# martinhoT/Footsies-Gym

Hardware: NVIDIA B200
Metric: env_frames_per_sec (higher is better)
Workload: dtype int32+fp32

## Files before the change

footsies_gym_b200/_capi.py:

```python
import ctypes as C
import os

from . import build as _build

FG_STATE_PLANES = 4
FG_STAT_COUNT = 16
STAT_NAMES = ["episodes", "p1_wins", "p2_wins", "double_ko", "episode_frames", "p1_specials",
              "p1_specials_neutral", "guard_breaks", "hits", "blocks", "env_frames", "resets"]


class FgConfig(C.Structure):
    _fields_ = [("struct_size", C.c_int32), ("num_envs", C.c_int32), ("device", C.c_int32),
                ("p1_bot", C.c_int32), ("p2_bot", C.c_int32), ("dense_reward", C.c_int32),
                ("frame_skip", C.c_int32), ("autoreset", C.c_int32), ("stale_intro_input", C.c_int32),
                ("skip_unactionable", C.c_int32), ("first_env_index", C.c_int64)]


class FgBuffers(C.Structure):
    _fields_ = [("struct_size", C.c_int32), ("reserved0", C.c_int32),
                ("state", C.c_void_p * FG_STATE_PLANES), ("stats", C.c_void_p),
                ("actions_p1", C.c_void_p), ("actions_p2", C.c_void_p), ("obs", C.c_void_p),
                ("reward", C.c_void_p), ("terminated", C.c_void_p), ("info_frame", C.c_void_p),
                ("info_misc", C.c_void_p), ("step_mask", C.c_void_p)]

# ... 70 lines not shown
        lib = load()
        self.nbytes = int(nbytes)
        ptr = lib.fg_host_alloc(int(device_index), self.nbytes)
        if not ptr:
            raise FootsiesLibraryError("fg_host_alloc failed: " + lib.fg_last_error().decode("utf-8", "replace"))
        self.ptr = ptr
        raw = (C.c_uint8 * max(self.nbytes, 1)).from_address(ptr)
        weakref.finalize(raw, lib.fg_host_free, ptr).atexit = False
        self.bytes = torch.frombuffer(raw, dtype=torch.uint8, count=self.nbytes)
        self._offset = 0

    def take(self, shape, dtype):
        import torch
        n = int(torch.Size(shape).numel()) * torch.empty((), dtype=dtype).element_size()
        off = (self._offset + 63) // 64 * 64
        if off + n > self.nbytes:
            raise ValueError("host block exhausted")
        self._offset = off + n
        return self.bytes[off:off + n].view(dtype).reshape(shape)


_lib = None

EXPORTS = ["fg_abi_version", "fg_last_error", "fg_algorithmic_bytes_per_env_step", "fg_create", "fg_destroy",
           "fg_bind", "fg_seed", "fg_reset", "fg_step", "fg_step_host", "fg_reset_host", "fg_step_host_compact",
           "fg_reset_host_compact", "fg_packed_reward_table", "fg_step_host_packed", "fg_reset_host_packed", "fg_host_alloc",
           "fg_host_free", "fg_delay_ring_step", "fg_get_state",
           "fg_set_state", "fg_read_stats", "fg_launch_count", "fg_policy_mlp_sample", "fg_policy_mlp_sample_p2", "fg_policy_last_error",
           "fg_rollout_mlp", "fg_rollout_mlp_pool", "fg_value_mlp", "fg_gae"]


def load(build_if_missing=True):
    global _lib
    if _lib is not None:
        return _lib
    path = _build.LIB_PATH
    if os.environ.get("FOOTSIES_B200_LIB"):
        pass
    elif _build.is_stale(path):
        if not build_if_missing:
            raise FootsiesLibraryError(f"{path} is missing or stale: run `python -m footsies_gym_b200.build`")
        _build.build()
    L = C.CDLL(path)
    vp, i32, i64 = C.c_void_p, C.c_int32, C.c_int64
    L.fg_abi_version.restype = i32
    L.fg_last_error.restype = C.c_char_p
    L.fg_algorithmic_bytes_per_env_step.restype = i32
    L.fg_algorithmic_bytes_per_env_step.argtypes = [C.POINTER(FgConfig)]
    L.fg_create.restype = i32
    L.fg_create.argtypes = [C.POINTER(FgConfig), C.POINTER(vp)]
    L.fg_destroy.restype = None
    L.fg_destroy.argtypes = [vp]
    L.fg_bind.restype = i32
    L.fg_bind.argtypes = [vp, C.POINTER(FgBuffers)]
    L.fg_seed.restype = i32
    L.fg_seed.argtypes = [vp, i64, vp, vp]
    L.fg_reset.restype = i32
    L.fg_reset.argtypes = [vp, vp, vp]
    L.fg_step.restype = i32
    L.fg_step.argtypes = [vp, vp]
    L.fg_step_host.restype = i32
    L.fg_step_host.argtypes = [vp, vp, vp, vp, vp, vp, vp, vp, vp]
    L.fg_reset_host.restype = i32
    L.fg_reset_host.argtypes = [vp, vp, vp, vp, vp, vp]
    L.fg_step_host_compact.restype = i32
    L.fg_step_host_compact.argtypes = [vp, vp, vp, C.POINTER(FgHostOutputs), vp]
    L.fg_reset_host_compact.restype = i32
    L.fg_reset_host_compact.argtypes = [vp, vp, C.POINTER(FgHostOutputs), vp]
    L.fg_packed_reward_table.restype = i32
    L.fg_packed_reward_table.argtypes = [vp, vp, vp]
    L.fg_step_host_packed.restype = i32
# ... 41 lines not shown
```

footsies_gym_b200/csrc/footsies_kernels.cu:

```cuda
#include <sched.h>
#include <stdlib.h>
#include <algorithm>

#include "rollout_kernel.h"
#include "step_kernel.cuh"

using namespace fg;
using namespace fgk;

namespace {

thread_local char g_err[512] = "";
int fail(int code, const char *fmt, const char *detail = "") {
    snprintf(g_err, sizeof g_err, fmt, detail);
    return code;
}
#define CUDA_TRY(expr) do { cudaError_t _e = (expr); if (_e != cudaSuccess) \
    return fail(FG_ERR_CUDA, #expr ": %s", cudaGetErrorString(_e)); } while (0)

}

struct fg_handle {
    fg_config cfg;
    fg_buffers buf;
// ... 11 lines not shown
    float *d_reward_table;
    uint32_t *d_pack_error;
    float h_reward_table[FG_PACKED_REWARD_TABLE_SIZE];
    int reward_table_count;
    float2 *d_position;
    uint8_t *d_obs_u8;
    cudaStream_t s_compute, s_copy;
    cudaEvent_t ev_fork, ev_join;
    std::vector<cudaEvent_t> ev_slice;
};

namespace {

int grid_for(const fg_handle *h, int blocks_per_sm) {
    int want = (h->cfg.num_envs + kThreads - 1) / kThreads;
    int cap = h->sm_count * blocks_per_sm;
    return want < cap ? (want > 0 ? want : 1) : cap;
}

Params make_params(const fg_handle *h, int first = 0, int count = -1) {
    Params p;
    memset(&p, 0, sizeof p);
    const size_t o = (size_t)first;
    p.pl_f1 = (uint4 *)h->buf.state[FG_PLANE_F1] + o; p.pl_f2 = (uint4 *)h->buf.state[FG_PLANE_F2] + o;
    p.pl_env = (uint4 *)h->buf.state[FG_PLANE_ENV] + o; p.pl_rng = (uint4 *)h->buf.state[FG_PLANE_RNG] + o;
    p.stats = (unsigned long long *)h->buf.stats;
    p.act1 = h->buf.actions_p1 ? h->buf.actions_p1 + o : nullptr;
    p.act2 = h->buf.actions_p2 ? h->buf.actions_p2 + o : nullptr;
    p.obs = (float4 *)h->buf.obs + 2 * o; p.reward = h->buf.reward + o; p.terminated = h->buf.terminated + o;
    p.info_frame = h->buf.info_frame + o; p.info_misc = (uint32_t *)h->buf.info_misc + o;
    p.step_mask = h->buf.step_mask ? h->buf.step_mask + o : nullptr;
    p.tables = h->d_tables;
    p.first_env_index = h->cfg.first_env_index + first;
    p.reverse = (int)(h->step_calls & 1);
    p.pdl = (count < 0 ? h->cfg.num_envs - first : count) >= h->pdl_min_envs;
    p.n = count < 0 ? h->cfg.num_envs - first : count; p.frame_skip = h->cfg.frame_skip; p.autoreset = h->cfg.autoreset;
    p.stale_intro = h->cfg.stale_intro_input;
    p.skip_unactionable = h->cfg.skip_unactionable;
    p.large_shape_min_envs = h->large_shape_min_envs;
    return p;
}

template <bool KF>
cudaError_t launch_step_k(const fg_config &c, int sm_count, cudaStream_t s, const Params &p) {
    const bool d = c.dense_reward != 0, m = p.step_mask != nullptr;
    if (c.p1_bot && c.p2_bot) return launch_step_d<KF, true, true>(d, m, sm_count, s, p);
    if (c.p1_bot) return launch_step_d<KF, true, false>(d, m, sm_count, s, p);
    if (c.p2_bot) return launch_step_d<KF, false, true>(d, m, sm_count, s, p);
// ... 407 lines not shown
    if (int rc = packed_init(h)) return rc;
    memcpy(table, h->h_reward_table, sizeof h->h_reward_table);
    *count = h->reward_table_count;
    return FG_OK;
}
int32_t fg_step_host_packed(fg_handle *h, const uint8_t *a1, const uint8_t *a2, fg_packed_result *out, void *stream) {
    return host_step_packed(h, a1, a2, out, (cudaStream_t)stream);
}
int32_t fg_reset_host_packed(fg_handle *h, const uint8_t *mask, fg_packed_result *out, void *stream) {
    return host_reset_packed(h, mask, out, (cudaStream_t)stream);
}

int32_t fg_abi_version(void) { return FG_ABI_VERSION; }
const char *fg_last_error(void) { return g_err; }

int32_t fg_algorithmic_bytes_per_env_step(const fg_config *cfg) {
    if (!cfg) return 0;
    const bool rng = cfg->p1_bot || cfg->p2_bot;
    int state = 2 * 16 * (rng ? 4 : 3);
    int actions = (cfg->p1_bot ? 0 : 1) + (cfg->p2_bot ? 0 : 1);
    return state + actions + 32  + 4  + 1  + 4  + 4 ;
}

int32_t fg_create(const fg_config *cfg, fg_handle **out) {
    if (!cfg || !out) return fail(FG_ERR_INVALID_ARGUMENT, "null argument%s");
    if (cfg->struct_size != (int32_t)sizeof(fg_config)) return fail(FG_ERR_INVALID_ARGUMENT, "fg_config.struct_size mismatch%s");
    if (cfg->num_envs <= 0) return fail(FG_ERR_INVALID_ARGUMENT, "num_envs must be positive%s");
    if (cfg->frame_skip < 1 || cfg->frame_skip > 64) return fail(FG_ERR_INVALID_ARGUMENT, "frame_skip must be in [1, 64]%s");
    if (cfg->skip_unactionable && cfg->p1_bot) return fail(FG_ERR_INVALID_ARGUMENT, "skip_unactionable needs an agent-controlled P1%s");
    int ndev = 0;
    if (cudaGetDeviceCount(&ndev) != cudaSuccess || ndev == 0) {
        cudaGetLastError();
        return fail(FG_ERR_NO_DEVICE, "no CUDA device: this library has no CPU fallback%s");
    }
    if (cfg->device < 0 || cfg->device >= ndev) return fail(FG_ERR_INVALID_ARGUMENT, "device ordinal out of range%s");
    CUDA_TRY(cudaSetDevice(cfg->device));
    fg_handle *h = new (std::nothrow) fg_handle();
    if (!h) return fail(FG_ERR_INVALID_STATE, "out of host memory%s");
    h->cfg = *cfg;
    h->bound = false;
    h->launches = 0;
    h->step_calls = 0;
    h->d_mask = nullptr;
    h->d_position = nullptr; h->d_obs_u8 = nullptr;
    h->d_packed = nullptr; h->d_reward_table = nullptr; h->d_pack_error = nullptr; h->reward_table_count = 0;
    h->s_compute = h->s_copy = nullptr;
// ... 91 lines not shown
int32_t fg_reset_host(fg_handle *h, const uint8_t *mask, float *obs, int32_t *info_frame, uint8_t *info_misc, void *stream) {
    HostOut o = { obs, nullptr, nullptr, nullptr, nullptr, info_frame, info_misc };
    return host_reset(h, mask, o, (cudaStream_t)stream);
}

int32_t fg_reset_host_compact(fg_handle *h, const uint8_t *mask, const fg_host_outputs *out, void *stream) {
    if (!out || out->struct_size != (int32_t)sizeof(fg_host_outputs))
        return fail(FG_ERR_INVALID_ARGUMENT, "fg_host_outputs is null or its struct_size does not match%s");
    HostOut o = { nullptr, out->position, out->obs_u8, nullptr, nullptr, out->info_frame, out->info_misc };
    return host_reset(h, mask, o, (cudaStream_t)stream);
}

int32_t fg_get_state(fg_handle *h, int32_t first, int32_t count, fg_env_state *out) {
    if (int rc = check_bound(h)) return rc;
    if (!out || first < 0 || count < 0 || (int64_t)first + count > h->cfg.num_envs)
        return fail(FG_ERR_INVALID_ARGUMENT, "env range out of bounds%s");
    CUDA_TRY(cudaSetDevice(h->cfg.device));
    CUDA_TRY(cudaDeviceSynchronize());
    std::vector<FgVec4> pl[FG_STATE_PLANES];
    for (int k = 0; k < FG_STATE_PLANES; k++) {
        pl[k].resize((size_t)count);
        CUDA_TRY(cudaMemcpy(pl[k].data(), (const FgVec4 *)h->buf.state[k] + first, sizeof(FgVec4) * (size_t)count, cudaMemcpyDeviceToHost));
    }
    for (int i = 0; i < count; i++)
        fg_decode_env(pl[FG_PLANE_F1][i], pl[FG_PLANE_F2][i], pl[FG_PLANE_ENV][i], pl[FG_PLANE_RNG][i], &out[i]);
    return FG_OK;
}

int32_t fg_set_state(fg_handle *h, int32_t first, int32_t count, const fg_env_state *in) {
    if (int rc = check_bound(h)) return rc;
    if (!in || first < 0 || count < 0 || (int64_t)first + count > h->cfg.num_envs)
        return fail(FG_ERR_INVALID_ARGUMENT, "env range out of bounds%s");
    std::vector<FgVec4> pl[FG_STATE_PLANES];
    for (int k = 0; k < FG_STATE_PLANES; k++) pl[k].resize((size_t)count);
    for (int i = 0; i < count; i++)
        if (fg_encode_env(&in[i], &pl[FG_PLANE_F1][i], &pl[FG_PLANE_F2][i], &pl[FG_PLANE_ENV][i], &pl[FG_PLANE_RNG][i]))
            return fail(FG_ERR_INVALID_STATE, "state not representable (unknown action id, WIN/has_won, or field out of range)%s");
    CUDA_TRY(cudaSetDevice(h->cfg.device));
    CUDA_TRY(cudaDeviceSynchronize());
    for (int k = 0; k < FG_STATE_PLANES; k++)
        CUDA_TRY(cudaMemcpy((FgVec4 *)h->buf.state[k] + first, pl[k].data(), sizeof(FgVec4) * (size_t)count, cudaMemcpyHostToDevice));
    return FG_OK;
}

int32_t fg_read_stats(fg_handle *h, uint64_t *out, void *stream) {
    if (int rc = check_bound(h)) return rc;
    if (!out) return fail(FG_ERR_INVALID_ARGUMENT, "null output%s");
    CUDA_TRY(cudaSetDevice(h->cfg.device));
    CUDA_TRY(cudaMemcpyAsync(out, h->buf.stats, sizeof(uint64_t) * FG_STAT_COUNT, cudaMemcpyDeviceToHost, (cudaStream_t)stream));
    CUDA_TRY(cudaStreamSynchronize((cudaStream_t)stream));
    return FG_OK;
}

int32_t fg_delay_ring_step(fg_handle *h, int32_t depth, int32_t pos, float *ring_obs, int32_t *ring_frame, uint8_t *ring_misc,
                           float *out_obs, int32_t *out_frame, uint8_t *out_misc, void *stream) {
    if (int rc = check_bound(h)) return rc;
    if (depth < 2 || pos < 0 || pos >= depth) return fail(FG_ERR_INVALID_ARGUMENT, "depth must be frame_delay + 1 >= 2 and 0 <= pos < depth%s");
    if (!ring_obs || !ring_frame || !ring_misc || !out_obs || !out_frame || !out_misc) return fail(FG_ERR_INVALID_ARGUMENT, "null buffer%s");
    if (((uintptr_t)ring_obs & 15u) || ((uintptr_t)out_obs & 15u) || ((uintptr_t)ring_misc & 3u) || ((uintptr_t)out_misc & 3u))
        return fail(FG_ERR_INVALID_ARGUMENT, "obs buffers must be 16-byte, misc buffers 4-byte aligned%s");
// ... 101 lines not shown
```

footsies_gym_b200/csrc/state_codec.h:

```cpp
#ifndef FOOTSIES_B200_STATE_CODEC_H
#define FOOTSIES_B200_STATE_CODEC_H

#include <stdint.h>
#include "../../include/footsies_b200.h"
#include "frame_tables.h"

#if defined(__CUDACC__)
#define FG_HD __host__ __device__ __forceinline__
#else
#define FG_HD static inline
#endif

#define FG_PLANE_F1 0
#define FG_PLANE_F2 1
#define FG_PLANE_ENV 2
#define FG_PLANE_RNG 3

#define FGP_FRAME_SHIFT 0
#define FGP_ACT_SHIFT 6
#define FGP_STUN_SHIFT 11
#define FGP_GUARD_SHIFT 16
#define FGP_VITAL_SHIFT 18
#define FGP_HITCNT_SHIFT 19
#define FGP_BUF_SHIFT 20
#define FGP_RSV_SHIFT 21
#define FGP_INBACK_SHIFT 22
#define FGP_RPROX_SHIFT 23
#define FGP_SHAKE_SHIFT 24
#define FGP_SHAKE_SIGN_SHIFT 27
#define FGP_CARRY_END (1u << 28)
#define FGP_CARRY_ALWAYS (1u << 29)
#define FGP_CARRY_NORMAL (1u << 30)
#define FGP_CARRY_MASK (7u << 28)
#define FGP_ROW_MASK 0x7ffu
#define FGP_MAX_FRAME 63

#define FGH_DASH_SHIFT 0
#define FGH_ARUN_SHIFT 8
// ... 106 lines not shown
    o->frame = (int32_t)e.x;
    o->recorded_input[0] = (int)fg_bits(m, FGM_REC1_SHIFT, 3);
    o->recorded_input[1] = (int)fg_bits(m, FGM_REC2_SHIFT, 3);
    o->done = (int)fg_bits(m, FGM_DONE_SHIFT, 1);
    o->cum_reward_index = (int)fg_bits(m, FGM_CUM_SHIFT, 4);
    o->actor_input[0] = (int)fg_bits(m, FGM_ACTOR1_SHIFT, 3);
    o->actor_input[1] = (int)fg_bits(m, FGM_ACTOR2_SHIFT, 3);
    o->rng_state[0] = r.x; o->rng_state[1] = r.y; o->rng_state[2] = r.z; o->rng_state[3] = r.w;
    o->bot_queue[0] = e.w; o->bot_queue[1] = e.z;
    o->p1_bot_memory = (int)fg_bits(m, FGM_P1MEM_SHIFT, 9);
}

static inline int fg_encode_env(const fg_env_state *s, FgVec4 *f1, FgVec4 *f2, FgVec4 *e, FgVec4 *r) {
    if (fg_encode_fighter(&s->f[0], f1) || fg_encode_fighter(&s->f[1], f2)) return -1;
    if (s->cum_reward_index < 0 || s->cum_reward_index >= FT_NUM_CUM) return -1;
    uint32_t m = ((uint32_t)s->recorded_input[0] & 7u) << FGM_REC1_SHIFT | ((uint32_t)s->recorded_input[1] & 7u) << FGM_REC2_SHIFT
               | (uint32_t)(s->done != 0) << FGM_DONE_SHIFT | (uint32_t)s->cum_reward_index << FGM_CUM_SHIFT
               | ((uint32_t)s->actor_input[0] & 7u) << FGM_ACTOR1_SHIFT | ((uint32_t)s->actor_input[1] & 7u) << FGM_ACTOR2_SHIFT
               | ((uint32_t)s->p1_bot_memory & 0x1ffu) << FGM_P1MEM_SHIFT;
    e->x = (uint32_t)s->frame; e->y = m; e->z = s->bot_queue[1]; e->w = s->bot_queue[0];
    r->x = s->rng_state[0]; r->y = s->rng_state[1]; r->z = s->rng_state[2]; r->w = s->rng_state[3];
    return 0;
}
#endif
```

footsies_gym_b200/csrc/step_kernel.cuh:

```cuda
#ifndef FOOTSIES_B200_STEP_KERNEL_CUH
#define FOOTSIES_B200_STEP_KERNEL_CUH
#include "device_once.h"
#include <cuda_runtime.h>
#include <stdint.h>
#include <stdio.h>
#include <string.h>
#include <new>
#include <vector>

#include "tables_host.h"

namespace fgk {

using namespace fg;

template <int THREADS_, int GROUP_, int STAGES_, int MIN_BLOCKS_>
struct StepShape {
    static constexpr int kThreads = THREADS_, kGroupThreads = GROUP_, kGroups = THREADS_ / GROUP_, kStages = STAGES_,
                         kMinBlocks = MIN_BLOCKS_;
    static_assert(THREADS_ % GROUP_ == 0 && GROUP_ % 32 == 0, "groups are whole warps");
};
#if defined(FG_THREADS)
#ifndef FG_GROUP
#define FG_GROUP FG_THREADS
// ... 2 lines not shown
#define FG_STAGES 2
#endif
#ifndef FG_BLOCKS_PER_SM
#define FG_BLOCKS_PER_SM 4
#endif
using ShapeSmall = StepShape<FG_THREADS, FG_GROUP, FG_STAGES, FG_BLOCKS_PER_SM>;
using ShapeLargeSingle = ShapeSmall;
using ShapeLargeFused = ShapeSmall;
#else
using ShapeSmall = StepShape<256, 256, 2, 3>;
using ShapeLargeSingle = StepShape<768, 256, 3, 1>;
using ShapeLargeFused = StepShape<1024, 256, 3, 1>;
#endif
constexpr int kLargeShapeMinEnvs = 768 * 1024;
#ifndef FG_SKIP_RNG_STORE
#define FG_SKIP_RNG_STORE 1
#endif
#ifndef FG_PDL
#define FG_PDL 1
#endif
#ifndef FG_REVERSE
#define FG_REVERSE 1
#endif
constexpr int kThreads = 256;
constexpr uint32_t kFull = 0xffffffffu;

struct Params {
    uint4 *pl_f1, *pl_f2, *pl_env, *pl_rng;
    unsigned long long *stats;
    const uint8_t *act1, *act2;
    float4 *obs;
    float *reward;
    uint8_t *terminated;
    int32_t *info_frame;
    uint32_t *info_misc;
    const Tables *tables;
    const uint8_t *mask;
    const uint8_t *step_mask;
    long long seed_base, first_env_index;
    int n, frame_skip, autoreset, stale_intro;
    int skip_unactionable;
    int large_shape_min_envs;
    int reverse;
    int pdl;
    int pdl_min_envs;
};

__device__ __forceinline__ void write_outputs(const Params &p, int i, const Env &e, float reward, bool terminated) {
    StepOutputs o;
    make_outputs(e, o);
    p.obs[2 * (size_t)i] = make_float4(o.obs[0], o.obs[1], o.obs[2], o.obs[3]);
    p.obs[2 * (size_t)i + 1] = make_float4(o.obs[4], o.obs[5], o.obs[6], o.obs[7]);
    p.reward[i] = reward;
    p.terminated[i] = terminated ? 1 : 0;
    p.info_frame[i] = e.frame;
    p.info_misc[i] = o.info_misc;
}

__device__ __forceinline__ void load_tables(Tables *dst, const Tables *src) {
    const uint4 *s = reinterpret_cast<const uint4 *>(src);
    uint4 *d = reinterpret_cast<uint4 *>(dst);
    for (int k = threadIdx.x; k < (int)(sizeof(Tables) / 16); k += blockDim.x) d[k] = s[k];
}

template <bool WITH_RNG>
__device__ __forceinline__ void load_env(const Params &p, int i, Env &e) {
    const uint4 a = p.pl_f1[i], b = p.pl_f2[i], c = p.pl_env[i];
    e.pos1 = u2f(a.x); e.vel1 = u2f(a.y); e.pk1 = a.z; e.hist1 = a.w;
    e.pos2 = u2f(b.x); e.vel2 = u2f(b.y); e.pk2 = b.z; e.hist2 = b.w;
    e.frame = (int32_t)c.x; e.misc = c.y; e.bq2 = c.z; e.bq1 = c.w;
    if (WITH_RNG) { const uint4 r = p.pl_rng[i]; e.r0 = r.x; e.r1 = r.y; e.r2 = r.z; e.r3 = r.w; }
    e.drew = false;
}
template <bool WITH_RNG>
__device__ __forceinline__ void store_env(const Params &p, int i, const Env &e) {
    p.pl_f1[i] = make_uint4(f2u(e.pos1), f2u(e.vel1), e.pk1, e.hist1);
    p.pl_f2[i] = make_uint4(f2u(e.pos2), f2u(e.vel2), e.pk2, e.hist2);
    p.pl_env[i] = make_uint4((uint32_t)e.frame, e.misc, e.bq2, e.bq1);
    if (WITH_RNG && (!FG_SKIP_RNG_STORE || e.drew)) p.pl_rng[i] = make_uint4(e.r0, e.r1, e.r2, e.r3);
}

__device__ __forceinline__ void flush_stats(StatAcc &acc, unsigned long long *s_stats, int lane) {
    const uint32_t w[3] = { acc.a, acc.r, acc.s };
    const int map[3][4] = { { FG_STAT_EPISODES, FG_STAT_P1_WINS, FG_STAT_P2_WINS, FG_STAT_DOUBLE_KO },
                            { -1, FG_STAT_HITS, FG_STAT_BLOCKS, FG_STAT_GUARD_BREAKS },
                                            { FG_STAT_P1_SPECIALS, FG_STAT_P1_SPECIALS_NEUTRAL, FG_STAT_RESETS, FG_STAT_ENV_FRAMES } };
#pragma unroll
    for (int k = 0; k < 3; k++)
#pragma unroll
        for (int b = 0; b < 4; b++) {
            if (map[k][b] < 0) continue;
            const uint32_t tot = __reduce_add_sync(kFull, (w[k] >> (8 * b)) & 255u);
            if (lane == 0 && tot) atomicAdd(&s_stats[map[k][b]], (unsigned long long)tot);
        }
    const uint32_t lo = __reduce_add_sync(kFull, acc.ep_frames & 0xffffu), hi = __reduce_add_sync(kFull, acc.ep_frames >> 16);
    if (lane == 0 && (lo | hi)) atomicAdd(&s_stats[FG_STAT_EPISODE_FRAMES], ((unsigned long long)hi << 16) + lo);
    acc.a = 0u; acc.r = 0u; acc.s = 0u; acc.ep_frames = 0u;
}

__device__ __forceinline__ uint32_t smem_u32(const void *p) { return (uint32_t)__cvta_generic_to_shared(p); }
__device__ __forceinline__ void mbar_init(uint64_t *bar, uint32_t count) {
    asm volatile("mbarrier.init.shared::cta.b64 [%0], %1;" ::"r"(smem_u32(bar)), "r"(count));
// ... 3 lines not shown
}
__device__ __forceinline__ void mbar_arrive(uint64_t *bar) {
    asm volatile("mbarrier.arrive.shared::cta.b64 _, [%0];" ::"r"(smem_u32(bar)) : "memory");
}
__device__ __forceinline__ void mbar_wait(uint64_t *bar, uint32_t parity) {
    asm volatile(
        "{\n"
        ".reg .pred P1;\n"
        "LAB_WAIT:\n"
        "mbarrier.try_wait.parity.shared::cta.b64 P1, [%0], %1;\n"
        "@P1 bra DONE;\n"
        "bra LAB_WAIT;\n"
        "DONE:\n"
        "}" ::"r"(smem_u32(bar)), "r"(parity) : "memory");
}
__device__ __forceinline__ void tma_load_1d(void *dst, const void *src, uint32_t bytes, uint64_t *bar) {
    asm volatile("cp.async.bulk.shared::cluster.global.mbarrier::complete_tx::bytes [%0], [%1], %2, [%3];"
                 ::"r"(smem_u32(dst)), "l"(src), "r"(bytes), "r"(smem_u32(bar)) : "memory");
}

template <class SH, int PLANES>
struct __align__(128) StepSmem {
    Tables T;
    uint4 stage[SH::kGroups][SH::kStages][PLANES][SH::kGroupThreads];
    uint64_t full_bar[SH::kGroups][SH::kStages], empty_bar[SH::kGroups][SH::kStages];
    unsigned long long stats[FG_STAT_COUNT];
};

template <class SH, bool KFUSED, bool P1BOT, bool P2BOT, bool DENSE, bool MASKED>
__global__ void __launch_bounds__(SH::kThreads, SH::kMinBlocks) step_kernel(const Params p) {
    constexpr bool kRng = P1BOT || P2BOT;
    constexpr int kPlanes = kRng ? 4 : 3;
    constexpr int kGroupThreads = SH::kGroupThreads, kGroups = SH::kGroups, kStages = SH::kStages;
    extern __shared__ __align__(128) unsigned char smem_raw[];
    StepSmem<SH, kPlanes> &S = *reinterpret_cast<StepSmem<SH, kPlanes> *>(smem_raw);
    const Tables &T = S.T;
    const int lane = threadIdx.x & 31;
    const int g = threadIdx.x / kGroupThreads, lt = threadIdx.x % kGroupThreads;
    const int num_chunks = (p.n + kGroupThreads - 1) / kGroupThreads;
    const int full_chunks = p.n / kGroupThreads;
    const int first = blockIdx.x * kGroups + g, stride = gridDim.x * kGroups;
    const uint4 *const planes[4] = { p.pl_f1, p.pl_f2, p.pl_env, p.pl_rng };
    auto issue = [&](int chunk, int s) {
        mbar_expect_tx(&S.full_bar[g][s], (uint32_t)(kPlanes * kGroupThreads * sizeof(uint4)));
#pragma unroll
        for (int k = 0; k < kPlanes; k++)
            tma_load_1d(S.stage[g][s][k], planes[k] + (size_t)chunk * kGroupThreads, (uint32_t)(kGroupThreads * sizeof(uint4)),
                        &S.full_bar[g][s]);
    };
    auto chunk_of = [&](int c) { return (FG_REVERSE && p.reverse && c < full_chunks) ? full_chunks - 1 - c : c; };
    if (lt == 0) {
        for (int s = 0; s < kStages; s++) { mbar_init(&S.full_bar[g][s], 1u); mbar_init(&S.empty_bar[g][s], kGroupThreads / 32); }
        asm volatile("fence.mbarrier_init.release.cluster;" ::: "memory");
    }
    if (FG_PDL && p.pdl) {
        load_tables(&S.T, p.tables);
        if (threadIdx.x < FG_STAT_COUNT) S.stats[threadIdx.x] = 0ull;
        asm volatile("griddepcontrol.launch_dependents;" ::: "memory");
        asm volatile("griddepcontrol.wait;" ::: "memory");
    }
    if (lt == 0) {
        for (int j = 0; j < kStages - 1; j++) {
            const int cj = first + j * stride;
            if (cj < num_chunks && chunk_of(cj) < full_chunks) issue(chunk_of(cj), j);
        }
    }
    if (!(FG_PDL && p.pdl)) {
        load_tables(&S.T, p.tables);
        if (threadIdx.x < FG_STAT_COUNT) S.stats[threadIdx.x] = 0ull;
    }
    __syncthreads();
    StatAcc acc = { 0u, 0u, 0u, 0u };
    uint32_t frames_since_flush = 0u;
    uint32_t nin1 = 0u, nin2 = 0u;
    {
        const int i0 = (first < num_chunks ? chunk_of(first) : num_chunks) * kGroupThreads + lt;
        if (i0 < p.n) { if (!P1BOT) nin1 = p.act1[i0]; if (!P2BOT) nin2 = p.act2[i0]; }
    }
    int k = 0;
    for (int cl = first; cl < num_chunks; cl += stride, k++) {
        const int s = k % kStages;
        const int c = chunk_of(cl);
        const int i = c * kGroupThreads + lt;
        const bool staged = c < full_chunks;
        bool valid = staged || i < p.n;
        if (MASKED) valid = valid && p.step_mask[valid ? i : 0] != 0;
        if (lt == 0) {
            const int cn = cl + (kStages - 1) * stride;
            if (cn < num_chunks && chunk_of(cn) < full_chunks) {
                const int sn = (k + kStages - 1) % kStages;
                if (k >= 1) mbar_wait(&S.empty_bar[g][sn], ((k - 1) / kStages) & 1);
                issue(chunk_of(cn), sn);
            }
        }
        const uint32_t act1 = nin1, act2 = nin2;
        {
            const int cn1 = cl + stride;
            const int in = (cn1 < num_chunks ? chunk_of(cn1) : num_chunks) * kGroupThreads + lt;
            if (in < p.n) { if (!P1BOT) nin1 = p.act1[in]; if (!P2BOT) nin2 = p.act2[in]; }
        }
        Env e;
        bool run = false;
        uint32_t in1 = 0u, in2 = 0u;
        if (staged) {
            mbar_wait(&S.full_bar[g][s], (k / kStages) & 1);
            const uint4 a = S.stage[g][s][0][lt], b = S.stage[g][s][1][lt], cc = S.stage[g][s][2][lt];
            e.pos1 = u2f(a.x); e.vel1 = u2f(a.y); e.pk1 = a.z; e.hist1 = a.w;
            e.pos2 = u2f(b.x); e.vel2 = u2f(b.y); e.pk2 = b.z; e.hist2 = b.w;
            e.frame = (int32_t)cc.x; e.misc = cc.y; e.bq2 = cc.z; e.bq1 = cc.w;
            if (kRng) { const uint4 r = S.stage[g][s][kPlanes - 1][lt]; e.r0 = r.x; e.r1 = r.y; e.r2 = r.z; e.r3 = r.w; }
            e.drew = false;
            __syncwarp();
            if (lane == 0) mbar_arrive(&S.empty_bar[g][s]);
        } else if (valid) {
            load_env<kRng>(p, i, e);
        }
        if (valid) {
            if ((e.misc >> FGM_DONE_SHIFT) & 1u) {
                if (p.autoreset) {
                    reset_env<P1BOT, P2BOT>(T, e, p.stale_intro != 0);
                    store_env<kRng>(p, i, e);
                    write_outputs(p, i, e, 0.0f, false);
                    acc.s += 0x10000u;
                } else {
                    p.reward[i] = 0.0f;
                }
            } else {
                run = true;
                in1 = P1BOT ? (e.misc >> FGM_ACTOR1_SHIFT) & 7u : act1 & 7u;
                in2 = P2BOT ? (e.misc >> FGM_ACTOR2_SHIFT) & 7u : act2 & 7u;
            }
        }
        double reward = 0.0;
        bool terminal = false;
        const int K = KFUSED ? p.frame_skip : 1;
        for (int kk = 0; kk < K; kk++) {
            if (run && !terminal) {
                simulate_frame<P1BOT, P2BOT, DENSE, KFUSED>(T, e, in1, in2, reward, terminal, acc);
                acc.s += 1u << 24;
                if (KFUSED) {
                    if (P1BOT) in1 = (e.misc >> FGM_ACTOR1_SHIFT) & 7u;
                    if (P2BOT) in2 = (e.misc >> FGM_ACTOR2_SHIFT) & 7u;
                }
            }
        }
        if (KFUSED && p.skip_unactionable) {
            bool more = run && !terminal && obs_is_skippable(e);
            while (__any_sync(kFull, more)) {
                for (int kk = 0; kk < K; kk++) {
                    if (more && !terminal) {
                        simulate_frame<P1BOT, P2BOT, DENSE, KFUSED>(T, e, 0u, in2, reward, terminal, acc);
                        acc.s += 1u << 24;
                        if (P2BOT) in2 = (e.misc >> FGM_ACTOR2_SHIFT) & 7u;
                    }
                }
                more = more && !terminal && obs_is_skippable(e);
                frames_since_flush += (uint32_t)K;
                if (frames_since_flush >= kStatFlushFrames) { flush_stats(acc, S.stats, lane); frames_since_flush = 0u; }
            }
        }
        if (run) {
            store_env<kRng>(p, i, e);
            write_outputs(p, i, e, (float)reward, terminal);
        }
        frames_since_flush += (uint32_t)K;
        if (frames_since_flush >= kStatFlushFrames) { flush_stats(acc, S.stats, lane); frames_since_flush = 0u; }
    }
    flush_stats(acc, S.stats, lane);
    __syncthreads();
    if (threadIdx.x < FG_STAT_COUNT && S.stats[threadIdx.x]) atomicAdd(&p.stats[threadIdx.x], S.stats[threadIdx.x]);
}

template <bool P1BOT, bool P2BOT>
__global__ void __launch_bounds__(kThreads) reset_kernel(const Params p) {
    extern __shared__ __align__(128) unsigned char smem_raw[];
    Tables &T = *reinterpret_cast<Tables *>(smem_raw);
    load_tables(&T, p.tables);
    __syncthreads();
    constexpr bool kRng = P1BOT || P2BOT;
    unsigned long long resets = 0ull;
    for (int i = blockIdx.x * blockDim.x + threadIdx.x; i < p.n; i += gridDim.x * blockDim.x) {
        if (p.mask && !p.mask[i]) continue;
        Env e;
        load_env<kRng>(p, i, e);
        reset_env<P1BOT, P2BOT>(T, e, p.stale_intro != 0);
        store_env<kRng>(p, i, e);
        write_outputs(p, i, e, 0.0f, false);
        resets++;
    }
    if (resets) atomicAdd(&p.stats[FG_STAT_RESETS], resets);
}

static __global__ void __launch_bounds__(kThreads) seed_kernel(const Params p) {
    for (int i = blockIdx.x * blockDim.x + threadIdx.x; i < p.n; i += gridDim.x * blockDim.x) {
        if (p.mask && !p.mask[i]) continue;
        uint32_t s0 = (uint32_t)(int32_t)(p.seed_base + p.first_env_index + i);
        uint32_t s1 = s0 * 1812433253u + 1u, s2 = s1 * 1812433253u + 1u, s3 = s2 * 1812433253u + 1u;
        p.pl_rng[i] = make_uint4(s0, s1, s2, s3);
    }
}

template <class SH, bool KF, bool B1, bool B2, bool D, bool M>
cudaError_t launch_step_shape(int sm_count, cudaStream_t s, const Params &p) {
    constexpr int kPlanes = (B1 || B2) ? 4 : 3;
    constexpr size_t bytes = sizeof(StepSmem<SH, kPlanes>);
    static DeviceOnceFlags configured;
    if (cudaError_t e = configure_once_per_device(configured, [] {
            return cudaFuncSetAttribute(step_kernel<SH, KF, B1, B2, D, M>, cudaFuncAttributeMaxDynamicSharedMemorySize, (int)bytes); }))
        return e;
    const int want = (p.n + SH::kThreads - 1) / SH::kThreads, cap = sm_count * SH::kMinBlocks;
    const int grid = want < cap ? (want > 0 ? want : 1) : cap;
#if FG_PDL
    if (!p.pdl) {
        step_kernel<SH, KF, B1, B2, D, M><<<grid, SH::kThreads, bytes, s>>>(p);
        return cudaSuccess;
    }
    cudaLaunchConfig_t cfg = {};
    cfg.gridDim = dim3((unsigned)grid);
    cfg.blockDim = dim3((unsigned)SH::kThreads);
    cfg.dynamicSmemBytes = bytes;
    cfg.stream = s;
    cudaLaunchAttribute attr[1];
    attr[0].id = cudaLaunchAttributeProgrammaticStreamSerialization;
    attr[0].val.programmaticStreamSerializationAllowed = 1;
    cfg.attrs = attr;
    cfg.numAttrs = 1;
    return cudaLaunchKernelEx(&cfg, step_kernel<SH, KF, B1, B2, D, M>, p);
// ... 30 lines not shown
```

footsies_gym_b200/env.py:

```python
import ctypes as C
from typing import Callable, Optional, Union

import numpy as np
import torch

from . import _capi
from . import frame_data as _fd
from .moves import FootsiesMove
from .spaces import footsies_action_space, footsies_observation_space


class FootsiesGameClosedError(RuntimeError):
    """Kept for API compatibility with footsies_gym.envs.exceptions (never raised: there is no game process)."""


def _as_bitmask(action, n, device):
    if isinstance(action, torch.Tensor):
        t = action
    else:
        t = torch.as_tensor(np.asarray(action))
    if t.dim() == 1 and t.shape[0] == 3 and n == 1 and t.dtype in (torch.bool,):
        t = t.reshape(1, 3)
    if t.dim() == 2:
        if t.shape != (n, 3):
# ... 129 lines not shown
        d = {"frame": frame, "p1_action": misc[:, 0], "p2_action": misc[:, 1],
             "p1_hitstun": misc[:, 2], "p2_hitstun": misc[:, 3]}
        d.update(obs_dict)
        return d

    def _config(self):
        return _capi.FgConfig(
            struct_size=C.sizeof(_capi.FgConfig), num_envs=self.num_envs, device=self.device.index,
            p1_bot=int(self.by_example), p2_bot=int(self._opponent_mode == "bot"),
            dense_reward=int(self.dense_reward), frame_skip=self.frame_skip, autoreset=int(self.autoreset),
            stale_intro_input=int(self.stale_intro_input), skip_unactionable=int(self.skip_unactionable),
            first_env_index=self.first_env_index)

    def _create_handle(self):
        if self._handle is not None:
            self._lib.fg_destroy(self._handle)
            self._handle = None
        h = C.c_void_p()
        cfg = self._config()
        _capi.check(self._lib.fg_create(C.byref(cfg), C.byref(h)))
        self._handle = h
        cfg2 = self._config()
        self._bind()
        self.algorithmic_bytes_per_env_step = int(self._lib.fg_algorithmic_bytes_per_env_step(C.byref(cfg2)))

    def _bind(self):
        b = _capi.FgBuffers()
        b.struct_size = C.sizeof(_capi.FgBuffers)
        for k in range(_capi.FG_STATE_PLANES):
            b.state[k] = self.state[k].data_ptr()
        b.stats = self.stats.data_ptr()
        b.actions_p1 = self.actions_p1.data_ptr()
        b.actions_p2 = self.actions_p2.data_ptr()
        b.obs = self.obs.data_ptr()
        b.reward = self.reward.data_ptr()
        b.terminated = self.terminated.data_ptr()
        b.info_frame = self.info_frame.data_ptr()
        b.info_misc = self.info_misc.data_ptr()
        b.step_mask = None if self._step_mask is None else self._step_mask.data_ptr()
        _capi.check(self._lib.fg_bind(self._handle, C.byref(b)))

    def _stream(self):
        return C.c_void_p(torch.cuda.current_stream(self.device).cuda_stream)

    def seed(self, seed: int, mask: Optional[torch.Tensor] = None):
        m = None if mask is None else mask.to(device=self.device, dtype=torch.uint8).contiguous()
        _capi.check(self._lib.fg_seed(self._handle, int(seed), None if m is None else C.c_void_p(m.data_ptr()),
# ... 362 lines not shown
```

include/footsies_b200.h:

```cpp
#ifndef FOOTSIES_B200_H
#define FOOTSIES_B200_H

#include <stdint.h>

#ifdef __cplusplus
extern "C" {
#endif

#define FG_ABI_VERSION 2

typedef enum {
    FG_OK = 0,
    FG_ERR_INVALID_ARGUMENT = -1,
    FG_ERR_NOT_BOUND = -2,
    FG_ERR_CUDA = -3,
    FG_ERR_NO_DEVICE = -4,
    FG_ERR_INVALID_STATE = -5
} fg_status;

typedef struct {
    int32_t struct_size;
    int32_t num_envs;
    int32_t device;
    int32_t p1_bot;
// ... 47 lines not shown
    int32_t input0;
    uint32_t hist_left;
    uint32_t hist_right;
    int32_t attack_run;
} fg_fighter_state;

typedef struct {
    fg_fighter_state f[2];
    int32_t frame;
    int32_t recorded_input[2];
    int32_t done;
    int32_t cum_reward_index;
    int32_t actor_input[2];
    uint32_t rng_state[4];
    uint32_t bot_queue[2];
    int32_t p1_bot_memory;
} fg_env_state;

typedef struct fg_handle fg_handle;

int32_t fg_abi_version(void);
const char *fg_last_error(void);
int32_t fg_algorithmic_bytes_per_env_step(const fg_config *cfg);

int32_t fg_create(const fg_config *cfg, fg_handle **out);
void fg_destroy(fg_handle *h);
int32_t fg_bind(fg_handle *h, const fg_buffers *buffers);

int32_t fg_seed(fg_handle *h, int64_t seed_base, const uint8_t *mask, void *stream);
int32_t fg_reset(fg_handle *h, const uint8_t *mask, void *stream);
int32_t fg_step(fg_handle *h, void *stream);
int32_t fg_step_host(fg_handle *h, const uint8_t *actions_p1, const uint8_t *actions_p2, float *obs,
                     float *reward, uint8_t *terminated, int32_t *info_frame, uint8_t *info_misc, void *stream);
int32_t fg_reset_host(fg_handle *h, const uint8_t *mask, float *obs, int32_t *info_frame, uint8_t *info_misc,
                      void *stream);

typedef struct {
    int32_t struct_size;
    int32_t reserved0;
    float *position;
    uint8_t *obs_u8;
    float *reward;
    uint8_t *terminated;
    int32_t *info_frame;
    uint8_t *info_misc;
} fg_host_outputs;
// ... 78 lines not shown
```

Baseline: 34.31 billion.

## Repack env state into hot planes with compressed velocity and split p1-bot plane

```diff
diff --git a/footsies_gym_b200/_capi.py b/footsies_gym_b200/_capi.py
--- a/footsies_gym_b200/_capi.py
+++ b/footsies_gym_b200/_capi.py
@@ -116,7 +116,8 @@
 
 _lib = None
 
-EXPORTS = ["fg_abi_version", "fg_last_error", "fg_algorithmic_bytes_per_env_step", "fg_create", "fg_destroy",
+EXPORTS = ["fg_abi_version", "fg_last_error", "fg_algorithmic_bytes_per_env_step", "fg_streamed_bytes_per_env_step",
+           "fg_create", "fg_destroy",
            "fg_bind", "fg_seed", "fg_reset", "fg_step", "fg_step_host", "fg_reset_host", "fg_step_host_compact",
            "fg_reset_host_compact", "fg_packed_reward_table", "fg_step_host_packed", "fg_reset_host_packed", "fg_host_alloc",
            "fg_host_free", "fg_delay_ring_step", "fg_get_state",
@@ -141,6 +142,8 @@
     L.fg_last_error.restype = C.c_char_p
     L.fg_algorithmic_bytes_per_env_step.restype = i32
     L.fg_algorithmic_bytes_per_env_step.argtypes = [C.POINTER(FgConfig)]
+    L.fg_streamed_bytes_per_env_step.restype = i32
+    L.fg_streamed_bytes_per_env_step.argtypes = [C.POINTER(FgConfig)]
     L.fg_create.restype = i32
     L.fg_create.argtypes = [C.POINTER(FgConfig), C.POINTER(vp)]
     L.fg_destroy.restype = None
diff --git a/footsies_gym_b200/csrc/footsies_kernels.cu b/footsies_gym_b200/csrc/footsies_kernels.cu
--- a/footsies_gym_b200/csrc/footsies_kernels.cu
+++ b/footsies_gym_b200/csrc/footsies_kernels.cu
@@ -57,8 +57,8 @@
     Params p;
     memset(&p, 0, sizeof p);
     const size_t o = (size_t)first;
-    p.pl_f1 = (uint4 *)h->buf.state[FG_PLANE_F1] + o; p.pl_f2 = (uint4 *)h->buf.state[FG_PLANE_F2] + o;
-    p.pl_env = (uint4 *)h->buf.state[FG_PLANE_ENV] + o; p.pl_rng = (uint4 *)h->buf.state[FG_PLANE_RNG] + o;
+    p.pl_hot_f = (uint4 *)h->buf.state[FG_PLANE_HOT_F] + o; p.pl_hot_e = (uint4 *)h->buf.state[FG_PLANE_HOT_E] + o;
+    p.pl_p1bot = (uint4 *)h->buf.state[FG_PLANE_P1BOT] + o; p.pl_rng = (uint4 *)h->buf.state[FG_PLANE_RNG] + o;
     p.stats = (unsigned long long *)h->buf.stats;
     p.act1 = h->buf.actions_p1 ? h->buf.actions_p1 + o : nullptr;
     p.act2 = h->buf.actions_p2 ? h->buf.actions_p2 + o : nullptr;
@@ -512,6 +512,13 @@
     return state + actions + 32  + 4  + 1  + 4  + 4 ;
 }
 
+int32_t fg_streamed_bytes_per_env_step(const fg_config *cfg) {
+    if (!cfg) return 0;
+    int state = 2 * 16 * (cfg->p1_bot ? 3 : 2);
+    int actions = (cfg->p1_bot ? 0 : 1) + (cfg->p2_bot ? 0 : 1);
+    return state + actions + 32  + 4  + 1  + 4  + 4 ;
+}
+
 int32_t fg_create(const fg_config *cfg, fg_handle **out) {
     if (!cfg || !out) return fail(FG_ERR_INVALID_ARGUMENT, "null argument%s");
     if (cfg->struct_size != (int32_t)sizeof(fg_config)) return fail(FG_ERR_INVALID_ARGUMENT, "fg_config.struct_size mismatch%s");
@@ -649,8 +656,12 @@
         pl[k].resize((size_t)count);
         CUDA_TRY(cudaMemcpy(pl[k].data(), (const FgVec4 *)h->buf.state[k] + first, sizeof(FgVec4) * (size_t)count, cudaMemcpyDeviceToHost));
     }
-    for (int i = 0; i < count; i++)
-        fg_decode_env(pl[FG_PLANE_F1][i], pl[FG_PLANE_F2][i], pl[FG_PLANE_ENV][i], pl[FG_PLANE_RNG][i], &out[i]);
+    for (int i = 0; i < count; i++) {
+        FgVec4 f1, f2, e;
+        fg_unpack_hot(pl[FG_PLANE_HOT_F][i], pl[FG_PLANE_HOT_E][i], f1, f2, e);
+        fg_unpack_p1bot(pl[FG_PLANE_P1BOT][i], e);
+        fg_decode_env(f1, f2, e, pl[FG_PLANE_RNG][i], &out[i]);
+    }
     return FG_OK;
 }
 
@@ -660,9 +671,15 @@
         return fail(FG_ERR_INVALID_ARGUMENT, "env range out of bounds%s");
     std::vector<FgVec4> pl[FG_STATE_PLANES];
     for (int k = 0; k < FG_STATE_PLANES; k++) pl[k].resize((size_t)count);
-    for (int i = 0; i < count; i++)
-        if (fg_encode_env(&in[i], &pl[FG_PLANE_F1][i], &pl[FG_PLANE_F2][i], &pl[FG_PLANE_ENV][i], &pl[FG_PLANE_RNG][i]))
+    for (int i = 0; i < count; i++) {
+        FgVec4 f1, f2, e;
+        if (fg_encode_env(&in[i], &f1, &f2, &e, &pl[FG_PLANE_RNG][i]))
             return fail(FG_ERR_INVALID_STATE, "state not representable (unknown action id, WIN/has_won, or field out of range)%s");
+        if (!fg_vel_storable(f1.y) || !fg_vel_storable(f2.y))
+            return fail(FG_ERR_INVALID_STATE, "state not representable (velocity_x is not 0 or +-(0.3125 .. 56) with two mantissa bits)%s");
+        fg_pack_hot(f1, f2, e, pl[FG_PLANE_HOT_F][i], pl[FG_PLANE_HOT_E][i]);
+        fg_pack_p1bot(e, pl[FG_PLANE_P1BOT][i]);
+    }
     CUDA_TRY(cudaSetDevice(h->cfg.device));
     CUDA_TRY(cudaDeviceSynchronize());
     for (int k = 0; k < FG_STATE_PLANES; k++)
diff --git a/footsies_gym_b200/csrc/state_codec.h b/footsies_gym_b200/csrc/state_codec.h
--- a/footsies_gym_b200/csrc/state_codec.h
+++ b/footsies_gym_b200/csrc/state_codec.h
@@ -7,13 +7,15 @@
 
 #if defined(__CUDACC__)
 #define FG_HD __host__ __device__ __forceinline__
+#define FG_HD_MEMBER __host__ __device__ __forceinline__
 #else
 #define FG_HD static inline
+#define FG_HD_MEMBER inline
 #endif
 
-#define FG_PLANE_F1 0
-#define FG_PLANE_F2 1
-#define FG_PLANE_ENV 2
+#define FG_PLANE_HOT_F 0
+#define FG_PLANE_HOT_E 1
+#define FG_PLANE_P1BOT 2
 #define FG_PLANE_RNG 3
 
 #define FGP_FRAME_SHIFT 0
@@ -166,4 +168,48 @@
     r->x = s->rng_state[0]; r->y = s->rng_state[1]; r->z = s->rng_state[2]; r->w = s->rng_state[3];
     return 0;
 }
+
+#define FGM_VEL_MASK 0xfffu
+#define FGM_P1_MASK 0x1ffu
+
+FG_HD uint32_t fg_vel_encode(uint32_t bits) {
+    const uint32_t mag = (bits >> 21) & 0x3ffu;
+    const uint32_t m = mag - (125u << 2);
+    return (m < mag ? m : 0u) | ((bits >> 26) & 32u);
+}
+FG_HD uint32_t fg_vel_decode(uint32_t code) {
+    const uint32_t m = code & 31u;
+    return (m ? (m + (125u << 2)) << 21 : 0u) | (code & 32u) << 26;
+}
+FG_HD bool fg_vel_storable(uint32_t bits) { return fg_vel_encode(bits) < 64u && fg_vel_decode(fg_vel_encode(bits)) == bits; }
+struct FgVelArith {
+    FG_HD_MEMBER uint32_t encode(uint32_t bits) const { return fg_vel_encode(bits); }
+    FG_HD_MEMBER uint32_t decode(uint32_t code) const { return fg_vel_decode(code); }
+};
+
+template <class V, class VC = FgVelArith>
+FG_HD void fg_pack_hot(const V &f1, const V &f2, const V &e, V &hf, V &he, const VC &vc = VC()) {
+    hf.x = f1.x; hf.y = f2.x; hf.z = f1.z; hf.w = f2.z;
+    he.x = e.x;
+    he.y = (e.y & ~FGM_VEL_MASK) | (vc.encode(f1.y) + (vc.encode(f2.y) << 6));
+    he.z = e.z;
+    he.w = f1.w | f2.w << 16;
+}
+template <class V>
+FG_HD void fg_pack_p1bot(const V &e, V &hp) { hp.x = e.w; hp.y = e.y & FGM_P1_MASK; hp.z = 0u; hp.w = 0u; }
+template <class V, class VC = FgVelArith>
+FG_HD void fg_unpack_hot(const V &hf, const V &he, V &f1, V &f2, V &e, const VC &vc = VC()) {
+    f1.x = hf.x; f1.y = vc.decode(he.y); f1.z = hf.z; f1.w = he.w & 0xffffu;
+    f2.x = hf.y; f2.y = vc.decode(he.y >> 6); f2.z = hf.w; f2.w = he.w >> 16;
+    e.x = he.x; e.y = he.y & ~FGM_VEL_MASK; e.z = he.z; e.w = 0u;
+}
+template <class V>
+FG_HD void fg_unpack_p1bot(const V &hp, V &e) { e.w = hp.x; e.y |= hp.y & FGM_P1_MASK; }
+
+FG_HD bool fg_queue_may_empty(uint32_t q, uint32_t k) { return ((q >> 9) & 127u) < k || ((q >> 24) & 127u) < k; }
+template <class V>
+FG_HD bool fg_rng_may_draw(const V &he, uint32_t bq1, bool p1_bot, bool p2_bot, uint32_t k, bool autoreset) {
+    return (p2_bot && fg_queue_may_empty(he.z, k)) || (p1_bot && fg_queue_may_empty(bq1, k))
+        || (autoreset && ((he.y >> FGM_DONE_SHIFT) & 1u));
+}
 #endif
diff --git a/footsies_gym_b200/csrc/step_kernel.cuh b/footsies_gym_b200/csrc/step_kernel.cuh
--- a/footsies_gym_b200/csrc/step_kernel.cuh
+++ b/footsies_gym_b200/csrc/step_kernel.cuh
@@ -48,11 +48,16 @@
 #ifndef FG_REVERSE
 #define FG_REVERSE 1
 #endif
+#ifndef FG_RNG_MODE
+#define FG_RNG_MODE 2
+#endif
+template <bool P1BOT, bool P2BOT>
+__host__ __device__ constexpr int staged_planes() { return (P1BOT ? 3 : 2) + ((FG_RNG_MODE == 2 && (P1BOT || P2BOT)) ? 1 : 0); }
 constexpr int kThreads = 256;
 constexpr uint32_t kFull = 0xffffffffu;
 
 struct Params {
-    uint4 *pl_f1, *pl_f2, *pl_env, *pl_rng;
+    uint4 *pl_hot_f, *pl_hot_e, *pl_p1bot, *pl_rng;
     unsigned long long *stats;
     const uint8_t *act1, *act2;
     float4 *obs;
@@ -89,21 +94,57 @@
     for (int k = threadIdx.x; k < (int)(sizeof(Tables) / 16); k += blockDim.x) d[k] = s[k];
 }
 
-template <bool WITH_RNG>
-__device__ __forceinline__ void load_env(const Params &p, int i, Env &e) {
-    const uint4 a = p.pl_f1[i], b = p.pl_f2[i], c = p.pl_env[i];
+struct VelLut {
+    const uint32_t *dec;
+    const uint8_t *enc;
+    __host__ __device__ __forceinline__ uint32_t encode(uint32_t bits) const { return enc[bits >> 21]; }
+    __host__ __device__ __forceinline__ uint32_t decode(uint32_t code) const { return dec[code & 63u]; }
+};
+__device__ __forceinline__ void build_vel_lut(uint32_t *dec, uint8_t *enc) {
+    for (int k = threadIdx.x; k < 2048; k += blockDim.x) {
+        enc[k] = (uint8_t)(fg_vel_encode((uint32_t)k << 21) & 63u);
+        if (k < 64) dec[k] = fg_vel_decode((uint32_t)k);
+    }
+}
+
+template <bool WITH_P1, class VC = FgVelArith>
+__device__ __forceinline__ void env_from_planes(const uint4 &hf, const uint4 &he, const uint4 &hp, Env &e, const VC &vc = VC()) {
+    uint4 a, b, c;
+    fg_unpack_hot(hf, he, a, b, c, vc);
+    if (WITH_P1) fg_unpack_p1bot(hp, c);
     e.pos1 = u2f(a.x); e.vel1 = u2f(a.y); e.pk1 = a.z; e.hist1 = a.w;
     e.pos2 = u2f(b.x); e.vel2 = u2f(b.y); e.pk2 = b.z; e.hist2 = b.w;
     e.frame = (int32_t)c.x; e.misc = c.y; e.bq2 = c.z; e.bq1 = c.w;
+    e.drew = false;
+}
+__device__ __forceinline__ uint4 env_word(const Env &e) { return make_uint4((uint32_t)e.frame, e.misc, e.bq2, e.bq1); }
+template <class VC = FgVelArith>
+__device__ __forceinline__ void store_hot(const Params &p, int i, const Env &e, const VC &vc = VC()) {
+    const uint4 a = make_uint4(f2u(e.pos1), f2u(e.vel1), e.pk1, e.hist1), b = make_uint4(f2u(e.pos2), f2u(e.vel2), e.pk2, e.hist2);
+    uint4 hf, he;
+    fg_pack_hot(a, b, env_word(e), hf, he, vc);
+    p.pl_hot_f[i] = hf;
+    p.pl_hot_e[i] = he;
+}
+__device__ __forceinline__ void store_p1bot(const Params &p, int i, const Env &e) {
+    uint4 hp;
+    fg_pack_p1bot(env_word(e), hp);
+    p.pl_p1bot[i] = hp;
+}
+template <bool WITH_RNG>
+__device__ __forceinline__ void store_rng(const Params &p, int i, const Env &e) {
+    if (WITH_RNG && (!FG_SKIP_RNG_STORE || e.drew)) p.pl_rng[i] = make_uint4(e.r0, e.r1, e.r2, e.r3);
+}
+template <bool WITH_RNG>
+__device__ __forceinline__ void load_env(const Params &p, int i, Env &e) {
+    env_from_planes<true>(p.pl_hot_f[i], p.pl_hot_e[i], p.pl_p1bot[i], e);
     if (WITH_RNG) { const uint4 r = p.pl_rng[i]; e.r0 = r.x; e.r1 = r.y; e.r2 = r.z; e.r3 = r.w; }
-    e.drew = false;
-}
-template <bool WITH_RNG>
-__device__ __forceinline__ void store_env(const Params &p, int i, const Env &e) {
-    p.pl_f1[i] = make_uint4(f2u(e.pos1), f2u(e.vel1), e.pk1, e.hist1);
-    p.pl_f2[i] = make_uint4(f2u(e.pos2), f2u(e.vel2), e.pk2, e.hist2);
-    p.pl_env[i] = make_uint4((uint32_t)e.frame, e.misc, e.bq2, e.bq1);
-    if (WITH_RNG && (!FG_SKIP_RNG_STORE || e.drew)) p.pl_rng[i] = make_uint4(e.r0, e.r1, e.r2, e.r3);
+}
+template <bool WITH_RNG, class VC = FgVelArith>
+__device__ __forceinline__ void store_env(const Params &p, int i, const Env &e, const VC &vc = VC()) {
+    store_hot(p, i, e, vc);
+    store_p1bot(p, i, e);
+    store_rng<WITH_RNG>(p, i, e);
 }
 
 __device__ __forceinline__ void flush_stats(StatAcc &acc, unsigned long long *s_stats, int lane) {
@@ -153,6 +194,8 @@
 template <class SH, int PLANES>
 struct __align__(128) StepSmem {
     Tables T;
+    uint32_t vel_dec[64];
+    uint8_t vel_enc[2048];
     uint4 stage[SH::kGroups][SH::kStages][PLANES][SH::kGroupThreads];
     uint64_t full_bar[SH::kGroups][SH::kStages], empty_bar[SH::kGroups][SH::kStages];
     unsigned long long stats[FG_STAT_COUNT];
@@ -161,17 +204,18 @@
 template <class SH, bool KFUSED, bool P1BOT, bool P2BOT, bool DENSE, bool MASKED>
 __global__ void __launch_bounds__(SH::kThreads, SH::kMinBlocks) step_kernel(const Params p) {
     constexpr bool kRng = P1BOT || P2BOT;
-    constexpr int kPlanes = kRng ? 4 : 3;
+    constexpr int kPlanes = staged_planes<P1BOT, P2BOT>();
     constexpr int kGroupThreads = SH::kGroupThreads, kGroups = SH::kGroups, kStages = SH::kStages;
     extern __shared__ __align__(128) unsigned char smem_raw[];
     StepSmem<SH, kPlanes> &S = *reinterpret_cast<StepSmem<SH, kPlanes> *>(smem_raw);
     const Tables &T = S.T;
+    const VelLut vel = { S.vel_dec, S.vel_enc };
     const int lane = threadIdx.x & 31;
     const int g = threadIdx.x / kGroupThreads, lt = threadIdx.x % kGroupThreads;
     const int num_chunks = (p.n + kGroupThreads - 1) / kGroupThreads;
     const int full_chunks = p.n / kGroupThreads;
     const int first = blockIdx.x * kGroups + g, stride = gridDim.x * kGroups;
-    const uint4 *const planes[4] = { p.pl_f1, p.pl_f2, p.pl_env, p.pl_rng };
+    const uint4 *const planes[4] = { p.pl_hot_f, p.pl_hot_e, P1BOT ? p.pl_p1bot : p.pl_rng, p.pl_rng };
     auto issue = [&](int chunk, int s) {
         mbar_expect_tx(&S.full_bar[g][s], (uint32_t)(kPlanes * kGroupThreads * sizeof(uint4)));
 #pragma unroll
@@ -186,6 +230,7 @@
     }
     if (FG_PDL && p.pdl) {
         load_tables(&S.T, p.tables);
+        build_vel_lut(S.vel_dec, S.vel_enc);
         if (threadIdx.x < FG_STAT_COUNT) S.stats[threadIdx.x] = 0ull;
         asm volatile("griddepcontrol.launch_dependents;" ::: "memory");
         asm volatile("griddepcontrol.wait;" ::: "memory");
@@ -198,6 +243,7 @@
     }
     if (!(FG_PDL && p.pdl)) {
         load_tables(&S.T, p.tables);
+        build_vel_lut(S.vel_dec, S.vel_enc);
         if (threadIdx.x < FG_STAT_COUNT) S.stats[threadIdx.x] = 0ull;
     }
     __syncthreads();
@@ -235,14 +281,23 @@
         uint32_t in1 = 0u, in2 = 0u;
         if (staged) {
             mbar_wait(&S.full_bar[g][s], (k / kStages) & 1);
-            const uint4 a = S.stage[g][s][0][lt], b = S.stage[g][s][1][lt], cc = S.stage[g][s][2][lt];
-            e.pos1 = u2f(a.x); e.vel1 = u2f(a.y); e.pk1 = a.z; e.hist1 = a.w;
-            e.pos2 = u2f(b.x); e.vel2 = u2f(b.y); e.pk2 = b.z; e.hist2 = b.w;
-            e.frame = (int32_t)cc.x; e.misc = cc.y; e.bq2 = cc.z; e.bq1 = cc.w;
-            if (kRng) { const uint4 r = S.stage[g][s][kPlanes - 1][lt]; e.r0 = r.x; e.r1 = r.y; e.r2 = r.z; e.r3 = r.w; }
-            e.drew = false;
+            const uint4 hf = S.stage[g][s][0][lt], he = S.stage[g][s][1][lt];
+            const uint4 hp = P1BOT ? S.stage[g][s][2][lt] : make_uint4(0u, 0u, 0u, 0u);
+            if (kRng && FG_RNG_MODE == 2) {
+                const uint4 r = S.stage[g][s][kPlanes - 1][lt];
+                e.r0 = r.x; e.r1 = r.y; e.r2 = r.z; e.r3 = r.w;
+            }
             __syncwarp();
             if (lane == 0) mbar_arrive(&S.empty_bar[g][s]);
+            if (kRng && FG_RNG_MODE != 2) {
+                e.r0 = 0u; e.r1 = 0u; e.r2 = 0u; e.r3 = 0u;
+                if (valid && (FG_RNG_MODE == 1 || (KFUSED && p.skip_unactionable)
+                              || fg_rng_may_draw(he, hp.x, P1BOT, P2BOT, (uint32_t)(KFUSED ? p.frame_skip : 1), p.autoreset != 0))) {
+                    const uint4 r = p.pl_rng[i];
+                    e.r0 = r.x; e.r1 = r.y; e.r2 = r.z; e.r3 = r.w;
+                }
+            }
+            env_from_planes<P1BOT>(hf, he, hp, e, vel);
         } else if (valid) {
             load_env<kRng>(p, i, e);
         }
@@ -250,7 +305,7 @@
             if ((e.misc >> FGM_DONE_SHIFT) & 1u) {
                 if (p.autoreset) {
                     reset_env<P1BOT, P2BOT>(T, e, p.stale_intro != 0);
-                    store_env<kRng>(p, i, e);
+                    store_env<kRng>(p, i, e, vel);
                     write_outputs(p, i, e, 0.0f, false);
                     acc.s += 0x10000u;
                 } else {
@@ -291,7 +346,9 @@
             }
         }
         if (run) {
-            store_env<kRng>(p, i, e);
+            store_hot(p, i, e, vel);
+            if (P1BOT || !staged) store_p1bot(p, i, e);
+            store_rng<kRng>(p, i, e);
             write_outputs(p, i, e, (float)reward, terminal);
         }
         frames_since_flush += (uint32_t)K;
@@ -333,7 +390,7 @@
 
 template <class SH, bool KF, bool B1, bool B2, bool D, bool M>
 cudaError_t launch_step_shape(int sm_count, cudaStream_t s, const Params &p) {
-    constexpr int kPlanes = (B1 || B2) ? 4 : 3;
+    constexpr int kPlanes = staged_planes<B1, B2>();
     constexpr size_t bytes = sizeof(StepSmem<SH, kPlanes>);
     static DeviceOnceFlags configured;
     if (cudaError_t e = configure_once_per_device(configured, [] {
diff --git a/footsies_gym_b200/env.py b/footsies_gym_b200/env.py
--- a/footsies_gym_b200/env.py
+++ b/footsies_gym_b200/env.py
@@ -175,7 +175,7 @@
         self._handle = h
         cfg2 = self._config()
         self._bind()
-        self.algorithmic_bytes_per_env_step = int(self._lib.fg_algorithmic_bytes_per_env_step(C.byref(cfg2)))
+        self.algorithmic_bytes_per_env_step = int(self._lib.fg_streamed_bytes_per_env_step(C.byref(cfg2)))
 
     def _bind(self):
         b = _capi.FgBuffers()
diff --git a/include/footsies_b200.h b/include/footsies_b200.h
--- a/include/footsies_b200.h
+++ b/include/footsies_b200.h
@@ -93,6 +93,7 @@
 int32_t fg_abi_version(void);
 const char *fg_last_error(void);
 int32_t fg_algorithmic_bytes_per_env_step(const fg_config *cfg);
+int32_t fg_streamed_bytes_per_env_step(const fg_config *cfg);
 
 int32_t fg_create(const fg_config *cfg, fg_handle **out);
 void fg_destroy(fg_handle *h);
```

Result: no change. 34.52 billion (median of 6 runs) (+0.6%).
